# VinAIResearch/COMBAT

Hardware: AMD Instinct MI355X
Metric: images/sec per alternated generator+surrogate step, CIFAR-10 bs=128, 1/2/4/8 GPU (higher is better)
Workload: dtype bf16; 1 GPU; train_generator.py --dataset cifar10 --pc 0.5 --noise_rate 0.08: alternated PreActResNet18 surrogate + UNet generator step (Phase C + Phase G, both Nesterov-SGD updates), bs=128 per GPU, on-device augmentation on; per_gpu_batch=128, global_batch=128, parallelism=dp1 (RCCL all-reduce of netC grads in Phase C, netG grads in Phase G), losses_finite=True, deterministic=True

## Files before the change

combat_amd/_lib.py:

```python
from __future__ import annotations

import ctypes as C
import os

HERE = os.path.dirname(os.path.abspath(__file__))
LIB_PATH = os.environ.get("COMBAT_HIP_LIB") or os.path.join(HERE, "libcombat_hip.so")

c_i32, c_i64, c_f32, c_vp = C.c_int32, C.c_int64, C.c_float, C.c_void_p


class ConvArgs(C.Structure):

    _fields_ = [
        ("N", c_i32), ("H", c_i32), ("W", c_i32), ("C", c_i32),
        ("P", c_i32), ("Q", c_i32), ("K", c_i32),
        ("R", c_i32), ("S", c_i32), ("stride", c_i32), ("pad", c_i32),
        ("mode", c_i32),
        ("src", c_vp), ("wpack", c_vp), ("kpad", c_i32), ("rows_pad", c_i32), ("dst", c_vp),
        ("pro_scale", c_vp), ("pro_shift", c_vp), ("pro_group_stride", c_i32), ("pro_act", c_i32),
        ("pro_slope", c_f32),
        ("bias", c_vp), ("add_pre", c_vp), ("mask_x", c_vp), ("mask_scale", c_vp), ("mask_shift", c_vp),
        ("mask_activated", c_i32), ("mask_group_stride", c_i32), ("mask_slope", c_f32), ("mask_mul_scale", c_i32),
        ("add_post", c_vp), ("tanh_out", c_i32),
        ("stats_kind", c_i32), ("stats", c_vp), ("xh_mean", c_vp), ("xh_rstd", c_vp),
        ("act_dst", c_vp), ("act_scale", c_vp), ("act_shift", c_vp), ("act_slope", c_f32),
        ("workspace", c_vp), ("workspace_bytes", c_i64),
        ("tile", c_i32),
        ("src2", c_vp), ("wpack2", c_vp), ("kpad2", c_i32), ("rows_pad2", c_i32),
        ("pro_act_dst", c_vp),
    ]


class WgradArgs(C.Structure):

    _fields_ = [
        ("N", c_i32), ("H", c_i32), ("W", c_i32), ("C", c_i32),
        ("P", c_i32), ("Q", c_i32), ("K", c_i32),
        ("R", c_i32), ("S", c_i32), ("stride", c_i32), ("pad", c_i32),
        ("src", c_vp), ("dy", c_vp), ("dw", c_vp), ("k_real", c_i32), ("c_real", c_i32),
        ("pro_scale", c_vp), ("pro_shift", c_vp), ("pro_group_stride", c_i32), ("pro_act", c_i32),
        ("pro_slope", c_f32), ("split", c_i32),
        ("workspace", c_vp), ("workspace_bytes", c_i64),
        ("defer_reduce", c_i32), ("reserved", c_i32),
        ("reduce_first", c_vp),
# ... 13 lines not shown
    _fields_ = [("gamma", c_vp), ("beta", c_vp), ("running_mean", c_vp), ("running_var", c_vp),
                ("scale", c_vp), ("shift", c_vp), ("C", c_i32), ("reserved", c_i32)]


SIGNATURES = {
    "combat_version": (C.c_char_p, []),
    "combat_abi_version": (C.c_int, []),
    "combat_set_deterministic": (None, [C.c_int]),
    "combat_get_deterministic": (C.c_int, []),
    "combat_conv_gemm": (C.c_int, [C.POINTER(ConvArgs), c_vp]),
    "combat_conv_gemm_pair": (C.c_int, [C.POINTER(ConvArgs), C.POINTER(ConvArgs), c_vp]),
    "combat_conv_workspace_bytes": (c_i64, [C.POINTER(ConvArgs)]),
    "combat_conv_pick_tile": (C.c_int, [C.POINTER(ConvArgs)]),
    "combat_conv_stats_granule": (C.c_int, [C.c_int]),
    "combat_conv_stats_layout": (C.c_int, [C.POINTER(ConvArgs), C.POINTER(c_i32), C.POINTER(c_i32)]),
    "combat_conv_wgrad": (C.c_int, [C.POINTER(WgradArgs), c_vp]),
    "combat_conv_wgrad_workspace_bytes": (c_i64, [C.POINTER(WgradArgs)]),
    "combat_conv_wgrad_reduce": (C.c_int, [C.POINTER(WgradArgs), c_vp]),
    "combat_pack_weights": (C.c_int, [c_vp, c_i32, c_i32, c_i32, c_i32, c_i32, c_vp, c_i32, c_i32, c_vp, c_i32,
                                      c_i32, c_vp]),
    "combat_norm_finalize": (C.c_int, [c_vp, c_i32, c_i32, c_i32, c_f32, c_f32, c_vp, c_vp, c_vp, c_vp, c_vp, c_vp,
                                       c_vp, c_vp, c_f32, c_vp, c_vp, c_i64, c_vp]),
    "combat_norm_scratch_bytes": (c_i64, [c_i32, c_i32]),
    "combat_bn_eval_fold": (C.c_int, [c_vp, c_vp, c_vp, c_vp, c_f32, c_i32, c_vp, c_vp, c_vp]),
    "combat_pack_weights_batch": (C.c_int, [c_vp, c_i32, c_vp]),
    "combat_bn_eval_fold_batch": (C.c_int, [c_vp, c_i32, c_f32, c_vp]),
    "combat_group_stats": (C.c_int, [c_vp, c_i32, c_i32, c_i32, c_vp, c_vp]),
    "combat_norm_bwd_finalize": (C.c_int, [c_vp, c_i32, c_i32, c_i32, c_f32, c_vp, c_vp, c_vp, c_vp, c_vp, c_vp,
                                           c_vp, c_vp, c_vp, c_i64, c_vp]),
    "combat_norm_bwd_apply": (C.c_int, [c_vp, c_vp, c_vp, c_vp, c_i64, c_i32, c_i32, c_i32, c_vp, c_vp, c_vp, c_vp]),
# ... 101 lines not shown
```

combat_amd/csrc/conv3x3_dma.hip:

```cpp
#include "conv_dma_epilogue.hpp"
#include <stdlib.h>

#ifdef COMBAT_STAMPS
static unsigned long long *g_stamps_dma_host = nullptr;
extern "C" int combat_debug_set_stamps_dma(void *p) { g_stamps_dma_host = (unsigned long long *)p; return 0; }
#define DSTAMP(k)                                                                                        \
    do {                                                                                                 \
        if (threadIdx.x == 0 && p.stamps) p.stamps[blockIdx.x * 16 + (k)] = __builtin_readcyclecounter(); \
        if (threadIdx.x == 0 && p.stamps && ((k) == 0 || (k) == 4)) p.stamps[blockIdx.x * 16 + 8 + (k)] = wall_clock64(); \
    } while (0)
#else
#define DSTAMP(k)
#endif

namespace {

typedef __attribute__((address_space(3))) void lds_void_t;

#if defined(COMBAT_ABL_NODMA)
#define ABL_DMA(x) 0
#else
#define ABL_DMA(x) (x)
#endif

// ... 453 lines not shown
    if constexpr (!WIDE) {
#ifndef COMBAT_ABL_NOTOUCH
        if constexpr (FLX >= 0) epi_touch<TE>(epi);
#endif
        block_barrier();
#ifdef COMBAT_ABL_NOEPI
        {
            float s = 0.f;
#pragma unroll
            for (int i = 0; i < T::FN; ++i)
#pragma unroll
                for (int j = 0; j < T::FM; ++j) s += acc[i][j][0] + acc[i][j][1] + acc[i][j][2] + acc[i][j][3];
            if (s == 12345.678f) reinterpret_cast<float *>(const_cast<void *>(a.dst))[lane] = s;
        }
#else
        if constexpr (FLX >= 0)
            epi_finish_fl<TE, kEpiFlavours[FLX < 0 ? 0 : FLX]>(epi, smem, acc, a, dst_bytes, lane, wid, n0, (long)tile_m * NW + wid, ragged,
                                                                 p.PQ, nullptr, EpiNoHook(), NW);
        else
            epi_finish<TE>(epi, smem, acc, a, dst_bytes, lane, wid, n0, (long)tile_m * NW + wid, ragged, p.PQ, p.flavour, NW);
#endif
    } else {
        epi_init<TE>(epi, lane, wid, n0, [&](int row) -> long { return tile_row_off(wid * 64 + (row - wid * 32)); });
        epi_fetch<TE>(epi, a, dst_bytes, lane, n0);
        block_barrier();
        f32x4_t half[T::FN][2];
#pragma unroll
        for (int i = 0; i < T::FN; ++i) {
            half[i][0] = acc[i][0];
            half[i][1] = acc[i][1];
        }
        epi_finish<TE>(epi, smem, half, a, dst_bytes, lane, wid, n0, ((long)tile_m * NW + wid) * 2, ragged, p.PQ, p.flavour);
// ... 7 lines not shown
        epi_finish<TE>(epi, smem, half, a, dst_bytes, lane, wid, n0, ((long)tile_m * NW + wid) * 2 + 1, ragged, p.PQ, p.flavour);
    }
    DSTAMP(4);
}

template <int BN, int TW, int HB, int NW, int RPW>
__global__ __launch_bounds__(64 * NW, NW == 8 || (RPW == 64 && HB == 2) ? 1 : 2)
void conv3x3_dma_kernel(const DmaParams p) {
    conv3x3_dma_body<BN, TW, HB, NW, RPW>(p);
}

template <int BN, int TW, int HB, int FLX>
__global__ __launch_bounds__(256, 2)
void conv3x3_dma_pro_kernel(const DmaParams p) {
    conv3x3_dma_body<BN, TW, HB, 4, 32, true, FLX>(p);
}

template <int FLI>
__device__ __forceinline__ void conv3x3_ws_body(const DmaParams &p) {
    constexpr int FL = FLI < 0 ? -1 : kEpiFlavours[FLI < 0 ? 0 : FLI];
    constexpr int BN = 64, TW = 16;
    using T = TileCfg<128, BN, 4>;
    using G = DGeo<TW, 4, 32>;
    using EC = EpiCfg<T>;
    constexpr int WBYTES = 9 * BN * 128, HBYTES = G::HBYTES, HPW = G::HPW, EPI_OFF = WBYTES + 2 * HBYTES;
    constexpr int TAB_OFF = EPI_OFF + EC::LDS_BYTES;
    static_assert(G::TI == 1 && G::TH == 8 && G::HWP == 18, "one 16 x 8 patch of one image per tile");
    extern __shared__ __attribute__((aligned(16))) unsigned char smem[];
    const combat_conv_args &a = p.a;
    const int tid = threadIdx.x, lane = tid & 63;
// ... 369 lines not shown
            return COMBAT_ELAUNCH;
        attr_set = true;
    }
    COMBAT_LAUNCH(kern, dim3(p.tiles_m * p.tiles_n), dim3(256), smem, st, p);
    CB_LAUNCH_CHECK();
    return COMBAT_OK;
}

template <int BN, int TW>
int launch_pro(const DmaParams &p, hipStream_t st) {
    if (p.flavour == 0) return p.nchunks == 1 ? launch_pro_fl<BN, TW, 1, 0>(p, st) : launch_pro_fl<BN, TW, 2, 0>(p, st);
    if (p.flavour == 2) return p.nchunks == 1 ? launch_pro_fl<BN, TW, 1, 2>(p, st) : launch_pro_fl<BN, TW, 2, 2>(p, st);
    return COMBAT_EINVAL;
}

template <int BN, int TW, int NW, int RPW = 32>
int launch(const combat_conv_args *a, hipStream_t st) {
    DmaParams p;
    fill<TW, NW, RPW>(a, BN, p);
    if (a->pro_scale) {
        if constexpr (NW == 4 && RPW == 32) return launch_pro<BN, TW>(p, st);
        else return COMBAT_EINVAL;
    }
    return p.nchunks == 1 ? launch_hb<BN, TW, 1, NW, RPW>(p, st) : launch_hb<BN, TW, 2, NW, RPW>(p, st);
}

int tile_bn(int tile) {
    return tile == COMBAT_TILE_D128x64 || tile == COMBAT_TILE_D256x64 || tile == COMBAT_TILE_D256W64 ? 64
                                                                                                 : (tile == COMBAT_TILE_D128x32 ? 32 : 0);
}
int tile_bm(int tile) { return tile == COMBAT_TILE_D256x64 || tile == COMBAT_TILE_D256W64 ? 256 : 128; }

int geo_th(const combat_conv_args *a, int bm) {
    const int tw = geo_tw(a);
// ... 57 lines not shown

int conv3x3d_pick(const combat_conv_args *a) {
    if (a->tile == COMBAT_TILE_S128x64) return ws_applicable(a) ? a->tile : 0;
    if (a->tile) {
        const int bn = tile_bn(a->tile);
        if (a->pro_scale && tile_bm(a->tile) != 128) return 0;
        if (a->tile == COMBAT_TILE_D256W64 && geo_tw(a) != 16) return 0;
        return bn && applicable(a, bn) && geo_th(a, tile_bm(a->tile)) ? a->tile : 0;
    }
    if (!applicable(a, 64)) return applicable(a, 32) ? COMBAT_TILE_D128x32 : 0;
    if (ws_applicable(a) && !getenv("COMBAT_NO_WS")) return COMBAT_TILE_S128x64;
    const long wgs64 = tiles_m_of(a) * (a->K / 64);
    return wgs64 <= 256 ? COMBAT_TILE_D128x32 : COMBAT_TILE_D128x64;
}

int conv3x3d_stats_layout(const combat_conv_args *a, int tile, int *rows, int *rows_per_image) {
    const bool per_wg = a->stats_kind & COMBAT_STATS_PER_WORKGROUP;
    if (tile == COMBAT_TILE_S128x64) {
        if (per_wg) {
            if (!ws_applicable(a)) return COMBAT_EINVAL;
            int per;
            ws_grid(tiles_m_of(a), per, *rows);
            *rows_per_image = 0;
            return COMBAT_OK;
        }
        tile = COMBAT_TILE_D128x64;
    }
    const int bn = tile_bn(tile);
    if (!bn || !applicable(a, bn)) return COMBAT_EINVAL;
    const int tw = geo_tw(a), bm = tile_bm(tile);
// ... 33 lines not shown
```

combat_amd/csrc/conv_common.hpp:

```cpp
#pragma once
#include "common.hpp"
#include <type_traits>

int conv3x3_pick(const combat_conv_args *a);
int conv3x3_stats_layout(const combat_conv_args *a, int tile, int *rows, int *rows_per_image);
int conv3x3_launch(const combat_conv_args *a, int tile, hipStream_t st);
int conv3x3d_pick(const combat_conv_args *a);
int conv3x3d_stats_layout(const combat_conv_args *a, int tile, int *rows, int *rows_per_image);
int conv3x3d_launch(const combat_conv_args *a, int tile, hipStream_t st);
int conv_gather_dma_bn(const combat_conv_args *a);
bool conv_gather_dma_parity_split(const combat_conv_args *a);
bool conv_c8_ok(const combat_conv_args *a);
int conv_c8_launch(const combat_conv_args *a, hipStream_t st);
bool conv_k8_ok(const combat_conv_args *a);
int conv_k8_launch(const combat_conv_args *a, hipStream_t st);
int conv_gather_dma_launch(const combat_conv_args *a, hipStream_t st);
int conv_gather_dma_pair_launch(const combat_conv_args *a, const combat_conv_args *b, hipStream_t st);
long conv_gather_dma_workspace(const combat_conv_args *a);
int conv_wgrad3x3_try(const combat_wgrad_args *a, hipStream_t st);
int conv_wgrad3x3_dma_try(const combat_wgrad_args *a, hipStream_t st);
long conv_wgrad3x3_dma_workspace(const combat_wgrad_args *a);
int conv_wgrad3x3_dma_reduce(const combat_wgrad_args *a, hipStream_t st);

template <int BM, int BN, int WGM_ = 0>
// ... 194 lines not shown
```

combat_amd/csrc/conv_dma_epilogue.hpp:

```cpp
#pragma once
#include "conv_common.hpp"

constexpr unsigned kDmaOob = 0x40000000u;

typedef __attribute__((address_space(3))) float lds_f32_t;
__device__ __forceinline__ void load8f_lds(const lds_f32_t *p, float (&v)[8]) {
    typedef __attribute__((address_space(3))) f32x4_t lds_f32x4_t;
    const f32x4_t a = *reinterpret_cast<const lds_f32x4_t *>(p);
    const f32x4_t b = *reinterpret_cast<const lds_f32x4_t *>(p + 4);
    v[0] = a[0]; v[1] = a[1]; v[2] = a[2]; v[3] = a[3];
    v[4] = b[0]; v[5] = b[1]; v[6] = b[2]; v[7] = b[3];
}

template <typename T>
struct EpiCfg {
    static constexpr int NC = T::NC;
    static constexpr int EQ = 32 * NC / 64;
    static constexpr int NPF = 3 * EQ + 4;
    static constexpr int EPW = 32 * T::EPS > 64 * 20 ? 32 * T::EPS : 64 * 20;
    static constexpr int LDS_BYTES = 4 * 4 * EPW;
};

template <typename T>
struct EpiRegs {
// ... 43 lines not shown
    asm volatile("" : "+v"(r.t_sc[0]), "+v"(r.t_sc[1]), "+v"(r.t_sh[0]), "+v"(r.t_sh[1]));
}

enum : int {
    EF_PRE = 1,
    EF_POST = 2,
    EF_MASK = 4,
    EF_MASK_TAB = 8,
    EF_MUL_SCALE = 16,
    EF_PER_IMAGE = 32,
    EF_ACT = 64,
    EF_STATS1 = 128,
    EF_STATS2 = 256,
    EF_BIAS = 512,
    EF_NODST = 1024,
};

__host__ __device__ inline int epi_flags_of(const combat_conv_args &a) {
    int f = 0;
    if (a.add_pre) f |= EF_PRE;
    if (a.add_post) f |= EF_POST;
    if (a.mask_x) {
        f |= EF_MASK;
        if (a.mask_scale && !a.mask_activated) f |= EF_MASK_TAB;
        if (a.mask_mul_scale && a.mask_scale) f |= EF_MUL_SCALE;
        if (a.mask_group_stride) f |= EF_PER_IMAGE;
    }
    if (a.act_dst) f |= EF_ACT;
    if ((a.stats_kind & 3) == 1) f |= EF_STATS1;
    if ((a.stats_kind & 3) == 2) f |= EF_STATS2;
    if (a.bias) f |= EF_BIAS;
    if (!a.dst) f |= EF_NODST;
    return f;
}

constexpr int kEpiRuntime = EF_PRE | EF_POST | EF_BIAS | EF_NODST;
constexpr int kEpiFlavours[] = {
    0,
    EF_ACT,
    EF_STATS1,
    EF_MASK | EF_MUL_SCALE,
    EF_MASK | EF_MASK_TAB | EF_STATS2,
};
constexpr int kNumEpiFlavours = sizeof(kEpiFlavours) / sizeof(int);

inline int epi_flavour_of(const combat_conv_args &a) {
    const int f = epi_flags_of(a) & ~kEpiRuntime;
    for (int i = 0; i < kNumEpiFlavours; ++i)
        if (kEpiFlavours[i] == f) return i;
    return -1;
}

struct EpiNoHook {
    __device__ __forceinline__ void operator()() const {}
};

template <typename T, int FL, typename PreStore = EpiNoHook, typename StatSink = EpiNoHook>
__device__ __forceinline__ void epi_finish_fl(EpiRegs<T> &er, unsigned char *smem, const f32x4_t (&acc)[T::FN][T::FM],
                                              const combat_conv_args &a, unsigned dst_bytes, int lane, int wid, int n0,
                                              long stats_row, bool ragged, int PQ, const lds_f32_t *lds_tabs = nullptr,
                                              PreStore pre_store = PreStore(), int wg_waves = 0,
                                              StatSink stat_sink = StatSink()) {
    constexpr int NC = EpiCfg<T>::NC, EQ = EpiCfg<T>::EQ, EPW = EpiCfg<T>::EPW;
    constexpr bool RT = FL < 0;
    const int fl = RT ? epi_flags_of(a) : (FL | (epi_flags_of(a) & kEpiRuntime));
    const bool has_pre = fl & EF_PRE, has_post = fl & EF_POST, has_mask = fl & EF_MASK, mask_tab = fl & EF_MASK_TAB;
    const bool mul_scale = fl & EF_MUL_SCALE, per_image = fl & EF_PER_IMAGE, has_act = fl & EF_ACT;
    const bool kind1 = fl & EF_STATS1, kind2 = fl & EF_STATS2, has_bias = fl & EF_BIAS, has_dst = !(fl & EF_NODST);
    const int fr = lane & 15, fq = lane >> 4, ec = lane % NC, K = a.K;
    const __amdgpu_buffer_rsrc_t r_dst = __builtin_amdgcn_make_buffer_rsrc(a.dst, 0, a.dst ? dst_bytes : 0u, 0x00020000);
    const __amdgpu_buffer_rsrc_t r_act = __builtin_amdgcn_make_buffer_rsrc(a.act_dst, 0, a.act_dst ? dst_bytes : 0u, 0x00020000);
    float *ep = reinterpret_cast<float *>(smem) + wid * EPW;
#pragma unroll
    for (int i = 0; i < T::FN; ++i)
#pragma unroll
        for (int j = 0; j < T::FM; ++j)
            *reinterpret_cast<f32x4_t *>(ep + (j * 16 + fr) * T::EPS + i * 16 + fq * 4) = acc[i][j];
    asm volatile("s_waitcnt lgkmcnt(0)" ::: "memory");

// ... 71 lines not shown
        if (has_act || kind1 || kind2) unpack8v(packed[q], vr);
        if (has_act) {
            float y[8];
#pragma unroll
            for (int e = 0; e < 8; ++e) {
                const float qa = fmaf(vr[e], tsc[e], tsh[e]);
                y[e] = qa > 0.f ? qa : qa * aslope;
            }
            packed_act[q] = pack8v(y);
        }
        if (kind1 || kind2) {
            if (ragged && er.evoff[q] == kDmaOob) {
#pragma unroll
                for (int e = 0; e < 8; ++e) vr[e] = 0.f;
            }
            if (kind2) {
#pragma unroll
                for (int e = 0; e < 8; ++e) {
                    s1[e] += vr[e];
                    s2[e] = fmaf(vr[e], (xm[e] - hmn[e]) * hrs[e], s2[e]);
                }
            } else {
#pragma unroll
                for (int e = 0; e < 8; ++e) {
                    s1[e] += vr[e];
                    s2[e] = fmaf(vr[e], vr[e], s2[e]);
                }
            }
        }
    }
    pre_store();
// ... 1 lines not shown
#pragma unroll
        for (int q = 0; q < EQ; ++q) __builtin_amdgcn_raw_buffer_store_b128(packed[q], r_dst, er.evoff[q], 0, 0);
    }
    if (has_act) {
#pragma unroll
        for (int q = 0; q < EQ; ++q) __builtin_amdgcn_raw_buffer_store_b128(packed_act[q], r_act, er.evoff[q], 0, 0);
    }
    if (kind1 || kind2) {
        constexpr bool kSink = !__is_same(StatSink, EpiNoHook);
        const bool per_wg = (kSink || wg_waves > 0) && (a.stats_kind & COMBAT_STATS_PER_WORKGROUP);
        constexpr int VPL = NC * 16 / 64;
        const int vg = (lane / NC) * VPL;
        float tot[VPL];
#pragma unroll
        for (int u = 0; u < VPL; ++u) tot[u] = 0.f;
        if (stats_row >= 0) {
            float *sp = ep + lane * 20;
            *reinterpret_cast<f32x4_t *>(sp) = f32x4_t{s1[0], s1[1], s1[2], s1[3]};
            *reinterpret_cast<f32x4_t *>(sp + 4) = f32x4_t{s1[4], s1[5], s1[6], s1[7]};
            *reinterpret_cast<f32x4_t *>(sp + 8) = f32x4_t{s2[0], s2[1], s2[2], s2[3]};
            *reinterpret_cast<f32x4_t *>(sp + 12) = f32x4_t{s2[4], s2[5], s2[6], s2[7]};
            asm volatile("s_waitcnt lgkmcnt(0)" ::: "memory");
#pragma unroll
            for (int src = 0; src < 64 / NC; ++src) {
                const float *rp = ep + (src * NC + ec) * 20 + vg;
#pragma unroll
                for (int u = 0; u < VPL; ++u) tot[u] += rp[u];
            }
        }
        if (!per_wg) {
            if (stats_row >= 0) {
                float *orow = a.stats + ((size_t)stats_row * 2 + (vg >> 3)) * K + n + (vg & 7);
#pragma unroll
                for (int u = 0; u < VPL; ++u) orow[u] = tot[u];
            }
        } else if constexpr (kSink) {
            stat_sink(tot);
        } else {
            float *slot = ep + lane * VPL;
#pragma unroll
            for (int u = 0; u < VPL; ++u) slot[u] = tot[u];
            __syncthreads();
            if (wid == 0) {
                float sum[VPL];
#pragma unroll
// ... 30 lines not shown
```

combat_amd/csrc/conv_gemm.hip:

```cpp
#include "conv_common.hpp"
#include "plan.hpp"
#include <stdlib.h>

namespace {

struct ConvParams {
    combat_conv_args a;
    int M;
    int PQ;
    int ntaps;
    int c_shift;
    int s_shift;
    int nkt;
    int tiles_m, tiles_n;
    int psplit;
    int mq;
    int cpt;
};

__device__ __forceinline__ int lds_off(int row, int kchunk) { return row * 128 + ((kchunk ^ ((row >> 1) & 7)) << 4); }

template <int BM, int BN>
__global__ __launch_bounds__(256) void conv_gemm_kernel(const ConvParams p) {
    using T = TileCfg<BM, BN>;
// ... 268 lines not shown
        if (bn) return bn == 64 ? COMBAT_TILE_G128x64 : COMBAT_TILE_G128x32;
        if (a->tile) return 0;
    }
    if (a->tile) return a->tile;
    const long M = (long)a->N * a->P * a->Q;
    if (a->K <= 16) return COMBAT_TILE_128x16;
    if (a->K % 128 != 0) return (M / 128) * ((a->K + 63) / 64) >= 256 ? COMBAT_TILE_128x64 : COMBAT_TILE_64x64;
    if ((M / 128) * (a->K / 128) >= 256) return COMBAT_TILE_128x128;
    if ((M / 64) * (a->K / 128) >= 256) return COMBAT_TILE_64x128;
    return COMBAT_TILE_64x64;
}

}

extern "C" int combat_conv_pick_tile(const combat_conv_args *a) { return a ? pick_tile(a) : COMBAT_EINVAL; }

extern "C" int64_t combat_conv_workspace_bytes(const combat_conv_args *a) {
    if (!a || (a->tile && a->tile != COMBAT_TILE_G128x64 && a->tile != COMBAT_TILE_G128x32)) return 0;
    return (int64_t)conv_gather_dma_workspace(a);
}

extern "C" int combat_conv_stats_granule(int tile) {
    switch (tile) {
        case COMBAT_TILE_H256x64: return 64;
        case COMBAT_TILE_128x128:
        case COMBAT_TILE_128x64:
        case COMBAT_TILE_128x16:
        case COMBAT_TILE_H128x128:
        case COMBAT_TILE_H128x64:
        case COMBAT_TILE_D128x64:
// ... 25 lines not shown
        gran = 128;
    const long M = (long)a->N * a->P * a->Q, PQ = (long)a->P * a->Q;
    *rows = (int)((M + gran - 1) / gran);
    *rows_per_image = (PQ % gran == 0) ? (int)(PQ / gran) : 0;
    const int bm = (tile == COMBAT_TILE_64x64 || tile == COMBAT_TILE_64x128) ? 64 : 128;
    if (tile == COMBAT_TILE_C8) {
    } else if (tile == COMBAT_TILE_G128x64 || tile == COMBAT_TILE_G128x32) {
        if (conv_gather_dma_parity_split(a)) *rows_per_image = 0;
    } else if (parity_split(*a) && (M / 4) % bm == 0) {
        *rows_per_image = 0;
    }
    return COMBAT_OK;
}

static int validate_conv_args(const combat_conv_args *a) {
    if (!a || !a->src || !a->wpack || (!a->dst && !a->act_dst)) return COMBAT_EINVAL;
    if (a->act_dst && (!a->act_scale || !a->act_shift)) return COMBAT_EINVAL;
    if (a->N <= 0 || a->H <= 0 || a->W <= 0 || a->P <= 0 || a->Q <= 0) return COMBAT_EINVAL;
    if (a->C < 8 || a->K < 8 || (a->K & 7)) return COMBAT_EINVAL;
    if (a->R != a->S || (a->R != 1 && a->R != 3)) return COMBAT_EINVAL;
    if (a->stride != 1 && a->stride != 2) return COMBAT_EINVAL;
    if (a->mode != 0 && a->mode != 1) return COMBAT_EINVAL;
    if (a->kpad <= 0 || (a->kpad & 63) || a->kpad < a->R * a->S * a->C) return COMBAT_EINVAL;
    if ((a->pro_scale == nullptr) != (a->pro_shift == nullptr)) return COMBAT_EINVAL;
    if (a->mask_scale && !a->mask_shift) return COMBAT_EINVAL;
    if (a->mask_mul_scale && !a->mask_scale) return COMBAT_EINVAL;
    if ((a->src2 == nullptr) != (a->wpack2 == nullptr)) return COMBAT_EINVAL;
    const int skind = a->stats_kind & 3;
    if (a->stats_kind < 0 || (a->stats_kind & ~(3 | COMBAT_STATS_PER_WORKGROUP)) || skind == 3 || (!skind && a->stats_kind) ||
        (skind && !a->stats))
        return COMBAT_EINVAL;
    if (skind == 2 && (!a->mask_x || !a->xh_mean || !a->xh_rstd)) return COMBAT_EINVAL;
    if (ilog2_exact(a->C) < 0) return COMBAT_EINVAL;
    if ((long)a->N * a->P * a->Q > 0x7fffffffL / 8) return COMBAT_EINVAL;
    return COMBAT_OK;
}

extern "C" int combat_conv_gemm(const combat_conv_args *a, void *stream);

extern "C" int combat_conv_gemm_pair(const combat_conv_args *a, const combat_conv_args *b, void *stream) {
    COMBAT_PLAN_HOOK(combat_conv_gemm_pair, a, b);
    if (validate_conv_args(a) != COMBAT_OK || validate_conv_args(b) != COMBAT_OK) return COMBAT_EINVAL;
    const int ta = pick_tile(a), tb = pick_tile(b);
    const bool gather = (ta == COMBAT_TILE_G128x64 || ta == COMBAT_TILE_G128x32) && ta == tb && !a->src2 && !b->src2;
    if (gather) {
        const int rc = conv_gather_dma_pair_launch(a, b, as_stream(stream));
        if (rc != 1) return rc;
// ... 37 lines not shown
```

combat_amd/engine.py:

```python
from __future__ import annotations

import ctypes
import os
from typing import Dict, List, Optional, Tuple

import torch

from . import ops
from ._lib import STATS_PER_WORKGROUP, TILE_D128x32, TILE_D128x64, TILE_S128x64, CombatHipError, ConvArgs, lib
from .nets import UNET_LAYERS
from .ops import Affine, PackedConv, bf16

BATCH_STATS_ROWS = 0 if os.environ.get("COMBAT_STATS_PER_WAVE") == "1" else STATS_PER_WORKGROUP

f32 = torch.float32


def _p(t):
    return None if t is None else t.data_ptr()


class Plan:

    serial = False
# ... 599 lines not shown
        plan.hold(a, part)
        plan.add(key + ".conv", lib.combat_conv_gemm, ctypes.byref(a))
        one_launch = act_dst is not None or defer
        if not fused and not (one_launch and pq <= self.FUSED_DIRECT_PX):
            g = _pow2_part(pq)
            parts = m // g
            part = slot.buf(key + ".part", (parts, 2, c), f32)
            plan.add(key + ".stats", lib.combat_group_stats, dst.data_ptr(), parts, g, c, part.data_ptr())
            rpg = pq // g
        rm = rv = nbt = None
        if running is not None:
            rm, rv, nbt = running
        plan.hold(gamma, beta, rm, rv, nbt)
        if one_launch:
            st.pending = dict(x=dst, part=part, rpg=rpg if part is not None else 0, pxg=m // groups, key=key,
                              gamma=gamma, beta=beta, rm=rm, rv=rv, nbt=nbt)
            if act_dst is not None:
                self._norm_act(plan, st, act_dst, slope)
            return st
        plan.add(key + ".finalize", lib.combat_norm_finalize, part.data_ptr(), groups, rpg, c, float(m // groups),
                 1e-5, _p(gamma), _p(beta), st.mean.data_ptr(), st.rstd.data_ptr(), st.scale.data_ptr(),
                 st.shift.data_ptr(), _p(rm), _p(rv), 0.1, _p(nbt), self._scratch.data_ptr(),
                 self._scratch.numel() * 4)
        return st

    def _lds_prologue_ok(self, src, pc: PackedConv) -> bool:
        if not FUSED_PROLOGUE or pc.R != 3 or pc.stride != 1:
            return False
        n, h, w, _ = src.shape
        probe = getattr(self, "_pro_probe", None)
        if probe is None:
# ... 2 lines not shown
        a = ConvArgs()
        a.N, a.H, a.W, a.C = src.shape
        a.P, a.Q, a.K = h, w, pc.Kc
        a.R = a.S = 3
        a.stride, a.pad, a.mode = 1, pc.pad, 0
        a.src, a.dst, a.pro_act_dst = src.data_ptr(), src.data_ptr(), src.data_ptr()
        a.wpack, a.kpad, a.rows_pad = pc.wf.data_ptr(), pc.kpad_f, pc.rows_f
        a.pro_scale, a.pro_shift, a.pro_act = probe.scale.data_ptr(), probe.shift.data_ptr(), 1
        return lib.combat_conv_pick_tile(ctypes.byref(a)) in (TILE_D128x64, TILE_D128x32)

    def _norm_act(self, plan: Plan, st: NormState, act_dst, slope: float):
        q = st.pending
        st.pending = None
        x = q["x"]
        plan.hold(x, act_dst, q["part"])
        plan.add(q["key"] + ".finact", lib.combat_norm_act_fused, x.data_ptr(), _p(q["part"]), st.groups, q["rpg"],
                 q["pxg"], st.C, 1e-5, float(slope), _p(q["gamma"]), _p(q["beta"]), st.mean.data_ptr(),
                 st.rstd.data_ptr(), st.scale.data_ptr(), st.shift.data_ptr(), _p(q["rm"]), _p(q["rv"]), 0.1,
                 _p(q["nbt"]), self._scratch.data_ptr(), self._scratch.numel() * 4, act_dst.data_ptr())

    def _dgrad_norm(self, plan: Plan, slot: Slot, key: str, dy, dz, pc: PackedConv, x_pre, st: NormState, *,
                    group_stride: int, slope: float, gamma=None, dgamma=None, dbeta=None, add_pre=None, shortcut=None):
        n, p, q, c = dz.shape
        pq, m = p * q, n * p * q
        groups = st.groups
        mask = Affine(st.scale, st.shift, group_stride, True, slope)
        a = ops.conv_args(dy, dz, pc, 1, add_pre=add_pre, mask_x=x_pre, mask=mask, workspace=plan.workspace(dy.device),
                          shortcut=shortcut)
        a.stats_kind = 2 | (BATCH_STATS_ROWS if groups == 1 else 0)
        a.xh_mean, a.xh_rstd = st.mean.data_ptr(), st.rstd.data_ptr()
        _tile_preference(a)
        rows, rpi = ops.conv_stats_layout(a)
        fused = (groups == 1) or (rpi > 0)
        part, rpg = None, 0
        if fused:
            part = slot.buf(key + ".bpart", (rows, 2, c), f32)
            a.stats = part.data_ptr()
            rpg = rows if groups == 1 else rpi
        else:
            a.stats_kind, a.xh_mean, a.xh_rstd = 0, None, None
        plan.hold(a, part)
        plan.add(key + ".dgrad", lib.combat_conv_gemm, ctypes.byref(a))
        if not fused and pq > self.FUSED_DIRECT_PX:
            part, rpg = self._stats_bwd(plan, slot, key, dz, x_pre, st)
        st.bpending = dict(part=part, rpg=rpg, gamma=gamma, dgamma=dgamma, dbeta=dbeta)

    def _stats_bwd(self, plan: Plan, slot: Slot, key: str, dz, x_pre, st: NormState):
        n, p, q, c = dz.shape
        pq, m = p * q, n * p * q
        g = _pow2_part(pq if st.groups > 1 else m)
        parts = m // g
        part = slot.buf(key + ".bpart", (parts, 2, c), f32)
        ppi = (pq // g) if st.groups > 1 else 0
        plan.add(key + ".bstats", lib.combat_group_stats_bwd, dz.data_ptr(), x_pre.data_ptr(), parts, g, c, ppi,
                 st.mean.data_ptr(), st.rstd.data_ptr(), part.data_ptr())
        return part, (pq // g if st.groups > 1 else parts)

    def _bwd_apply(self, plan: Plan, slot: Slot, key: str, dz, x_pre, dx, st: NormState, add=None):
        n, p, q, c = dz.shape
        pq, m = p * q, n * p * q
        pend = getattr(st, "bpending", None) or dict(part=None, rpg=0, gamma=None, dgamma=None, dbeta=None)
        st.bpending = None
        part, rpg = pend["part"], pend["rpg"]
        pxg = m // st.groups
        if part is None and (st.groups == 1 or pq > self.FUSED_DIRECT_PX):
            part, rpg = self._stats_bwd(plan, slot, key, dz, x_pre, st)
        plan.hold(dz, x_pre, dx, add, part, pend["gamma"], pend["dgamma"], pend["dbeta"])
        plan.add(key + ".bfused", lib.combat_norm_bwd_fused, dz.data_ptr(), x_pre.data_ptr(), _p(add), _p(part),
                 st.groups, rpg, pxg, c, _p(pend["gamma"]), st.mean.data_ptr(), st.rstd.data_ptr(),
                 _p(pend["dgamma"]), _p(pend["dbeta"]), self._scratch.data_ptr(), self._scratch.numel() * 4,
                 dx.data_ptr())




class _BN:
    def __init__(self, eng: "NetEngine", mod: torch.nn.BatchNorm2d, prefix: str):
        self.prefix, self.C = prefix, mod.num_features
        self.gamma, self.beta = mod.weight.data, mod.bias.data
# ... 958 lines not shown
```

include/combat_hip.h:

```cpp
#ifndef COMBAT_HIP_H
#define COMBAT_HIP_H

#include <stdint.h>

#ifdef __cplusplus
extern "C" {
#endif

#define COMBAT_OK 0
#define COMBAT_EINVAL (-1)
#define COMBAT_ELAUNCH (-2)

const char *combat_version(void);
int combat_abi_version(void);

void combat_set_deterministic(int on);
int combat_get_deterministic(void);

typedef struct combat_conv_args {
    int32_t N, H, W, C;
    int32_t P, Q, K;
    int32_t R, S, stride, pad;
    int32_t mode;
    const void *src;
// ... 15 lines not shown
    int32_t mask_mul_scale;
    const void *add_post;
    int32_t tanh_out;
    int32_t stats_kind;
    float *stats;
    const float *xh_mean, *xh_rstd;
    void *act_dst;
    const float *act_scale, *act_shift;
    float act_slope;
    void *workspace;
    int64_t workspace_bytes;
    int32_t tile;
    const void *src2, *wpack2;
    int32_t kpad2, rows_pad2;
    void *pro_act_dst;
} combat_conv_args;

#define COMBAT_STATS_PER_WORKGROUP 4
#define COMBAT_TILE_128x128 1
#define COMBAT_TILE_128x64 2
#define COMBAT_TILE_64x64 3
#define COMBAT_TILE_128x16 4
#define COMBAT_TILE_64x128 5
#define COMBAT_TILE_H256x64 6
#define COMBAT_TILE_H128x128 7
#define COMBAT_TILE_H128x64 8
#define COMBAT_TILE_H64x64 9
#define COMBAT_TILE_D128x64 10
#define COMBAT_TILE_D128x32 11
#define COMBAT_TILE_G128x64 12
#define COMBAT_TILE_G128x32 13
#define COMBAT_TILE_D256x64 14
#define COMBAT_TILE_C8 15
#define COMBAT_TILE_S128x64 17
#define COMBAT_TILE_K8 18
#define COMBAT_TILE_D256W64 16

int combat_conv_gemm(const combat_conv_args *a, void *stream);
int combat_conv_gemm_pair(const combat_conv_args *a, const combat_conv_args *b, void *stream);
int64_t combat_conv_workspace_bytes(const combat_conv_args *a);
int combat_conv_pick_tile(const combat_conv_args *a);
int combat_conv_stats_granule(int tile);
int combat_conv_stats_layout(const combat_conv_args *a, int32_t *rows, int32_t *rows_per_image);

typedef struct combat_wgrad_args {
    int32_t N, H, W, C;
    int32_t P, Q, K;
    int32_t R, S, stride, pad;
    const void *src;
    const void *dy;
    float *dw;
    int32_t k_real;
    int32_t c_real;
    const float *pro_scale, *pro_shift;
    int32_t pro_group_stride;
    int32_t pro_act;
    float pro_slope;
    int32_t split;
// ... 188 lines not shown
```

Measured before the change: 33340 images/sec.

## Fuse InstanceNorm stats, normalize and activation into whole-image conv epilogue

```diff
diff --git a/combat_amd/_lib.py b/combat_amd/_lib.py
--- a/combat_amd/_lib.py
+++ b/combat_amd/_lib.py
@@ -28,6 +28,8 @@
         ("tile", c_i32),
         ("src2", c_vp), ("wpack2", c_vp), ("kpad2", c_i32), ("rows_pad2", c_i32),
         ("pro_act_dst", c_vp),
+        ("ln_act_dst", c_vp), ("ln_mean", c_vp), ("ln_rstd", c_vp), ("ln_scale", c_vp), ("ln_shift", c_vp),
+        ("ln_dx", c_vp), ("ln_eps", c_f32), ("ln_slope", c_f32),
     ]
 
 
@@ -71,6 +73,7 @@
     "combat_conv_pick_tile": (C.c_int, [C.POINTER(ConvArgs)]),
     "combat_conv_stats_granule": (C.c_int, [C.c_int]),
     "combat_conv_stats_layout": (C.c_int, [C.POINTER(ConvArgs), C.POINTER(c_i32), C.POINTER(c_i32)]),
+    "combat_conv_norm_local": (C.c_int, [C.POINTER(ConvArgs)]),
     "combat_conv_wgrad": (C.c_int, [C.POINTER(WgradArgs), c_vp]),
     "combat_conv_wgrad_workspace_bytes": (c_i64, [C.POINTER(WgradArgs)]),
     "combat_conv_wgrad_reduce": (C.c_int, [C.POINTER(WgradArgs), c_vp]),
diff --git a/combat_amd/csrc/conv3x3_dma.hip b/combat_amd/csrc/conv3x3_dma.hip
--- a/combat_amd/csrc/conv3x3_dma.hip
+++ b/combat_amd/csrc/conv3x3_dma.hip
@@ -491,8 +491,11 @@
             if (s == 12345.678f) reinterpret_cast<float *>(const_cast<void *>(a.dst))[lane] = s;
         }
 #else
-        if constexpr (FLX >= 0)
-            epi_finish_fl<TE, kEpiFlavours[FLX < 0 ? 0 : FLX]>(epi, smem, acc, a, dst_bytes, lane, wid, n0, (long)tile_m * NW + wid, ragged,
+        if constexpr (FLX >= 100)
+            epi_finish_fl<TE, FLX == 100 ? kEpiLocalFwd : kEpiLocalBwd, EpiNoHook, EpiNoHook, TW>(
+                epi, smem, acc, a, dst_bytes, lane, wid, n0, (long)tile_m * NW + wid, ragged, p.PQ, nullptr, EpiNoHook(), NW);
+        else if constexpr (FLX >= 0)
+            epi_finish_fl<TE, kEpiFlavours[FLX < 0 || FLX >= kNumEpiFlavours ? 0 : FLX]>(epi, smem, acc, a, dst_bytes, lane, wid, n0, (long)tile_m * NW + wid, ragged,
                                                                  p.PQ, nullptr, EpiNoHook(), NW);
         else
             epi_finish<TE>(epi, smem, acc, a, dst_bytes, lane, wid, n0, (long)tile_m * NW + wid, ragged, p.PQ, p.flavour, NW);
@@ -530,6 +533,13 @@
 __global__ __launch_bounds__(256, 2)
 void conv3x3_dma_pro_kernel(const DmaParams p) {
     conv3x3_dma_body<BN, TW, HB, 4, 32, true, FLX>(p);
+}
+
+template <int BN, int TW, int HB, int DIR>
+__global__ __launch_bounds__(256, 2)
+void conv3x3_dma_ln_kernel(const DmaParams p) {
+    static_assert(DGeo<TW, 4, 32>::WHOLE, "a workgroup owns whole images");
+    conv3x3_dma_body<BN, TW, HB, 4, 32, false, 100 + DIR>(p);
 }
 
 template <int FLI>
@@ -929,10 +939,39 @@
     return COMBAT_EINVAL;
 }
 
+template <int BN, int TW, int HB, int DIR>
+int launch_ln_hb(const DmaParams &p, hipStream_t st) {
+    using G = DGeo<TW, 4, 32>;
+    constexpr int stage = HB * G::HBYTES + 3 * BN * 128 + 1024;
+    constexpr int ep = EpiCfg<TileCfg<128, BN, 4>>::LDS_BYTES * (TW == 4 && DIR == 1 ? 2 : 1);
+    constexpr int smem = stage > ep ? stage : ep;
+    static_assert(2 * smem <= 160 * 1024, "two workgroups per CU");
+    auto kern = conv3x3_dma_ln_kernel<BN, TW, HB, DIR>;
+    static bool attr_set = false;
+    if (!attr_set) {
+        if (hipFuncSetAttribute(reinterpret_cast<const void *>(kern), hipFuncAttributeMaxDynamicSharedMemorySize, smem) != hipSuccess)
+            return COMBAT_ELAUNCH;
+        attr_set = true;
+    }
+    COMBAT_LAUNCH(kern, dim3(p.tiles_m * p.tiles_n), dim3(256), smem, st, p);
+    CB_LAUNCH_CHECK();
+    return COMBAT_OK;
+}
+
+template <int BN, int TW>
+int launch_ln(const DmaParams &p, hipStream_t st) {
+    if (p.a.mode == 0) return p.nchunks == 1 ? launch_ln_hb<BN, TW, 1, 0>(p, st) : launch_ln_hb<BN, TW, 2, 0>(p, st);
+    return p.nchunks == 1 ? launch_ln_hb<BN, TW, 1, 1>(p, st) : launch_ln_hb<BN, TW, 2, 1>(p, st);
+}
+
 template <int BN, int TW, int NW, int RPW = 32>
 int launch(const combat_conv_args *a, hipStream_t st) {
     DmaParams p;
     fill<TW, NW, RPW>(a, BN, p);
+    if (a->ln_act_dst || a->ln_dx) {
+        if constexpr (NW == 4 && RPW == 32 && (TW == 4 || TW == 8)) return conv3x3d_norm_local(a) ? launch_ln<BN, TW>(p, st) : COMBAT_EINVAL;
+        else return COMBAT_EINVAL;
+    }
     if (a->pro_scale) {
         if constexpr (NW == 4 && RPW == 32) return launch_pro<BN, TW>(p, st);
         else return COMBAT_EINVAL;
@@ -1020,6 +1059,15 @@
     return wgs64 <= 256 ? COMBAT_TILE_D128x32 : COMBAT_TILE_D128x64;
 }
 
+bool conv3x3d_norm_local(const combat_conv_args *a) {
+    const int tw = geo_tw(a);
+    if ((tw != 4 && tw != 8) || a->tile == COMBAT_TILE_D256x64 || !(applicable(a, 64) || applicable(a, 32))) return false;
+    if (a->pro_scale || a->pro_act_dst || a->act_dst || a->src2) return false;
+    if (a->mode == 0) return !a->mask_x && (a->stats_kind & 3) != 2;
+    return a->mask_x && a->mask_scale && a->mask_shift && !a->mask_activated && !a->mask_mul_scale &&
+           a->mask_group_stride == a->K && (a->stats_kind & 3) != 1;
+}
+
 int conv3x3d_stats_layout(const combat_conv_args *a, int tile, int *rows, int *rows_per_image) {
     const bool per_wg = a->stats_kind & COMBAT_STATS_PER_WORKGROUP;
     if (tile == COMBAT_TILE_S128x64) {
diff --git a/combat_amd/csrc/conv_common.hpp b/combat_amd/csrc/conv_common.hpp
--- a/combat_amd/csrc/conv_common.hpp
+++ b/combat_amd/csrc/conv_common.hpp
@@ -6,6 +6,7 @@
 int conv3x3_stats_layout(const combat_conv_args *a, int tile, int *rows, int *rows_per_image);
 int conv3x3_launch(const combat_conv_args *a, int tile, hipStream_t st);
 int conv3x3d_pick(const combat_conv_args *a);
+bool conv3x3d_norm_local(const combat_conv_args *a);
 int conv3x3d_stats_layout(const combat_conv_args *a, int tile, int *rows, int *rows_per_image);
 int conv3x3d_launch(const combat_conv_args *a, int tile, hipStream_t st);
 int conv_gather_dma_bn(const combat_conv_args *a);
diff --git a/combat_amd/csrc/conv_dma_epilogue.hpp b/combat_amd/csrc/conv_dma_epilogue.hpp
--- a/combat_amd/csrc/conv_dma_epilogue.hpp
+++ b/combat_amd/csrc/conv_dma_epilogue.hpp
@@ -81,6 +81,7 @@
     EF_STATS2 = 256,
     EF_BIAS = 512,
     EF_NODST = 1024,
+    EF_LOCAL = 2048,
 };
 
 __host__ __device__ inline int epi_flags_of(const combat_conv_args &a) {
@@ -110,6 +111,8 @@
     EF_MASK | EF_MASK_TAB | EF_STATS2,
 };
 constexpr int kNumEpiFlavours = sizeof(kEpiFlavours) / sizeof(int);
+constexpr int kEpiLocalFwd = EF_STATS1 | EF_LOCAL;
+constexpr int kEpiLocalBwd = EF_MASK | EF_MASK_TAB | EF_PER_IMAGE | EF_STATS2 | EF_LOCAL;
 
 inline int epi_flavour_of(const combat_conv_args &a) {
     const int f = epi_flags_of(a) & ~kEpiRuntime;
@@ -122,7 +125,7 @@
     __device__ __forceinline__ void operator()() const {}
 };
 
-template <typename T, int FL, typename PreStore = EpiNoHook, typename StatSink = EpiNoHook>
+template <typename T, int FL, typename PreStore = EpiNoHook, typename StatSink = EpiNoHook, int LTW = 0>
 __device__ __forceinline__ void epi_finish_fl(EpiRegs<T> &er, unsigned char *smem, const f32x4_t (&acc)[T::FN][T::FM],
                                               const combat_conv_args &a, unsigned dst_bytes, int lane, int wid, int n0,
                                               long stats_row, bool ragged, int PQ, const lds_f32_t *lds_tabs = nullptr,
@@ -130,6 +133,9 @@
                                               StatSink stat_sink = StatSink()) {
     constexpr int NC = EpiCfg<T>::NC, EQ = EpiCfg<T>::EQ, EPW = EpiCfg<T>::EPW;
     constexpr bool RT = FL < 0;
+    constexpr bool kLocal = !RT && (FL & EF_LOCAL) != 0, kLocal4 = kLocal && LTW == 4, kLocalBwd = kLocal && (FL & EF_STATS2) != 0;
+    static_assert(!kLocal || LTW == 4 || LTW == 8, "local InstanceNorm: whole-image tiles");
+    float *const ep2 = reinterpret_cast<float *>(smem) + (4 + wid) * EPW;
     const int fl = RT ? epi_flags_of(a) : (FL | (epi_flags_of(a) & kEpiRuntime));
     const bool has_pre = fl & EF_PRE, has_post = fl & EF_POST, has_mask = fl & EF_MASK, mask_tab = fl & EF_MASK_TAB;
     const bool mul_scale = fl & EF_MUL_SCALE, per_image = fl & EF_PER_IMAGE, has_act = fl & EF_ACT;
@@ -231,7 +237,19 @@
 #pragma unroll
                 for (int e = 0; e < 8; ++e) vr[e] = 0.f;
             }
-            if (kind2) {
+            if constexpr (kLocal4) {
+                float *tp = ep + r * T::EPS + ec * 8;
+                *reinterpret_cast<f32x4_t *>(tp) = f32x4_t{vr[0], vr[1], vr[2], vr[3]};
+                *reinterpret_cast<f32x4_t *>(tp + 4) = f32x4_t{vr[4], vr[5], vr[6], vr[7]};
+                if constexpr (kLocalBwd) {
+                    float pr[8];
+#pragma unroll
+                    for (int e = 0; e < 8; ++e) pr[e] = fmaf(vr[e], (xm[e] - hmn[e]) * hrs[e], 0.f);
+                    float *pp = ep2 + r * T::EPS + ec * 8;
+                    *reinterpret_cast<f32x4_t *>(pp) = f32x4_t{pr[0], pr[1], pr[2], pr[3]};
+                    *reinterpret_cast<f32x4_t *>(pp + 4) = f32x4_t{pr[4], pr[5], pr[6], pr[7]};
+                }
+            } else if (kind2) {
 #pragma unroll
                 for (int e = 0; e < 8; ++e) {
                     s1[e] += vr[e];
@@ -263,7 +281,7 @@
         float tot[VPL];
 #pragma unroll
         for (int u = 0; u < VPL; ++u) tot[u] = 0.f;
-        if (stats_row >= 0) {
+        if (!kLocal4 && stats_row >= 0) {
             float *sp = ep + lane * 20;
             *reinterpret_cast<f32x4_t *>(sp) = f32x4_t{s1[0], s1[1], s1[2], s1[3]};
             *reinterpret_cast<f32x4_t *>(sp + 4) = f32x4_t{s1[4], s1[5], s1[6], s1[7]};
@@ -277,7 +295,101 @@
                 for (int u = 0; u < VPL; ++u) tot[u] += rp[u];
             }
         }
-        if (!per_wg) {
+        if constexpr (kLocal) {
+            constexpr int BN = NC * 8, NK = kLocalBwd ? 3 : 2;
+            constexpr int ITEMS = LTW == 4 ? 2 * BN / 64 : 1;
+            const float countf = (float)PQ;
+            double t1[ITEMS], t2[ITEMS];
+            float *cf = ep + 512;
+            if constexpr (LTW == 4) {
+#pragma unroll
+                for (int k = 0; k < ITEMS; ++k) {
+                    const int id = lane + 64 * k, h = id / BN, ch = id % BN;
+                    t1[k] = t2[k] = 0.0;
+#pragma unroll
+                    for (int i = 0; i < 16; ++i) {
+                        const float v = ep[(h * 16 + i) * T::EPS + ch];
+                        t1[k] += (double)v;
+                        if constexpr (kLocalBwd) t2[k] += (double)ep2[(h * 16 + i) * T::EPS + ch];
+                        else t2[k] += (double)fmaf(v, v, 0.f);
+                    }
+                }
+                cf = ep;
+            } else {
+                float *slot = ep + lane * VPL;
+#pragma unroll
+                for (int u = 0; u < VPL; ++u) slot[u] = tot[u];
+                asm volatile("s_waitcnt lgkmcnt(0)" ::: "memory");
+                __builtin_amdgcn_s_barrier();
+                asm volatile("" ::: "memory");
+                const float *p0 = reinterpret_cast<const float *>(smem) + (wid & ~1) * EPW, *p1 = p0 + EPW;
+                const int c = (lane % BN) >> 3, e = lane & 7;
+                const int i1 = ((e / VPL) * NC + c) * VPL + e % VPL, i2 = (((8 + e) / VPL) * NC + c) * VPL + (8 + e) % VPL;
+                t1[0] = (double)p0[i1] + (double)p1[i1];
+                t2[0] = (double)p0[i2] + (double)p1[i2];
+            }
+#pragma unroll
+            for (int k = 0; k < ITEMS; ++k) {
+                const int id = lane + 64 * k, h = LTW == 4 ? id / BN : 0, ch = id % BN;
+                const long img = (stats_row * 32 + h * 16) / PQ;
+                const bool own = id < (LTW == 4 ? 2 : 1) * BN;
+                const bool pub = own && img < a.N && (LTW == 4 || !(wid & 1));
+                const long o = img * K + n0 + ch;
+                float *cp = cf + h * NK * BN + ch;
+                if constexpr (!kLocalBwd) {
+                    const double mean = t1[k] / countf;
+                    double var = t2[k] / countf - mean * mean;
+                    if (var < 0.0) var = 0.0;
+                    const double rstd = 1.0 / sqrt(var + (double)a.ln_eps);
+                    const float fsc = (float)rstd, fsh = (float)(0.0 - mean * rstd);
+                    if (own) {
+                        cp[0] = fsc;
+                        cp[BN] = fsh;
+                    }
+                    if (pub) {
+                        a.ln_mean[o] = (float)mean;
+                        a.ln_rstd[o] = (float)rstd;
+                        a.ln_scale[o] = fsc;
+                        a.ln_shift[o] = fsh;
+                    }
+                } else {
+                    const bool ok = own && img < a.N;
+                    const double mean = ok ? (double)a.xh_mean[o] : 0.0, rstd = ok ? (double)a.xh_rstd[o] : 1.0;
+                    const double m1 = t1[k] / countf, m2 = t2[k] / countf;
+                    if (own) {
+                        cp[0] = (float)rstd;
+                        cp[BN] = (float)(-rstd * rstd * m2);
+                        cp[2 * BN] = (float)(rstd * (mean * rstd * m2 - m1));
+                    }
+                    (void)pub;
+                }
+            }
+            asm volatile("s_waitcnt lgkmcnt(0)" ::: "memory");
+            const float lslope = a.ln_slope;
+            const __amdgpu_buffer_rsrc_t r_out = __builtin_amdgcn_make_buffer_rsrc(kLocalBwd ? a.ln_dx : a.ln_act_dst, 0, dst_bytes, 0x00020000);
+#pragma unroll
+            for (int q = 0; q < EQ; ++q) {
+                const int h = LTW == 4 ? q * 2 / EQ : 0;
+                float k0[8], k1[8], vr[8], y[8];
+                load8f(cf + (h * NK + 0) * BN + ec * 8, k0);
+                load8f(cf + (h * NK + 1) * BN + ec * 8, k1);
+                unpack8v(packed[q], vr);
+                if constexpr (kLocalBwd) {
+                    float k2[8], xm[8];
+                    load8f(cf + (h * NK + 2) * BN + ec * 8, k2);
+                    unpack8v(er.e_x[q], xm);
+#pragma unroll
+                    for (int e = 0; e < 8; ++e) y[e] = fmaf(k0[e], vr[e], fmaf(k1[e], xm[e], k2[e]));
+                } else {
+#pragma unroll
+                    for (int e = 0; e < 8; ++e) {
+                        const float qa = fmaf(vr[e], k0[e], k1[e]);
+                        y[e] = qa > 0.f ? qa : qa * lslope;
+                    }
+                }
+                __builtin_amdgcn_raw_buffer_store_b128(pack8v(y), r_out, er.evoff[q], 0, 0);
+            }
+        } else if (!per_wg) {
             if (stats_row >= 0) {
                 float *orow = a.stats + ((size_t)stats_row * 2 + (vg >> 3)) * K + n + (vg & 7);
 #pragma unroll
diff --git a/combat_amd/csrc/conv_gemm.hip b/combat_amd/csrc/conv_gemm.hip
--- a/combat_amd/csrc/conv_gemm.hip
+++ b/combat_amd/csrc/conv_gemm.hip
@@ -306,6 +306,12 @@
 }
 
 extern "C" int combat_conv_pick_tile(const combat_conv_args *a) { return a ? pick_tile(a) : COMBAT_EINVAL; }
+
+static bool conv_norm_local(const combat_conv_args *a) {
+    const int tile = pick_tile(a);
+    return (tile == COMBAT_TILE_D128x64 || tile == COMBAT_TILE_D128x32) && conv3x3d_norm_local(a);
+}
+extern "C" int combat_conv_norm_local(const combat_conv_args *a) { return a && conv_norm_local(a) ? 1 : 0; }
 
 extern "C" int64_t combat_conv_workspace_bytes(const combat_conv_args *a) {
     if (!a || (a->tile && a->tile != COMBAT_TILE_G128x64 && a->tile != COMBAT_TILE_G128x32)) return 0;
@@ -361,7 +367,7 @@
 }
 
 static int validate_conv_args(const combat_conv_args *a) {
-    if (!a || !a->src || !a->wpack || (!a->dst && !a->act_dst)) return COMBAT_EINVAL;
+    if (!a || !a->src || !a->wpack || (!a->dst && !a->act_dst && !a->ln_dx)) return COMBAT_EINVAL;
     if (a->act_dst && (!a->act_scale || !a->act_shift)) return COMBAT_EINVAL;
     if (a->N <= 0 || a->H <= 0 || a->W <= 0 || a->P <= 0 || a->Q <= 0) return COMBAT_EINVAL;
     if (a->C < 8 || a->K < 8 || (a->K & 7)) return COMBAT_EINVAL;
@@ -378,6 +384,12 @@
         (skind && !a->stats))
         return COMBAT_EINVAL;
     if (skind == 2 && (!a->mask_x || !a->xh_mean || !a->xh_rstd)) return COMBAT_EINVAL;
+    if (a->ln_act_dst || a->ln_dx) {
+        if (skind || !conv_norm_local(a)) return COMBAT_EINVAL;
+        if (a->mode == 0 ? (a->ln_dx || !a->dst || !a->ln_mean || !a->ln_rstd || !a->ln_scale || !a->ln_shift)
+                         : (a->ln_act_dst || !a->xh_mean || !a->xh_rstd))
+            return COMBAT_EINVAL;
+    }
     if (ilog2_exact(a->C) < 0) return COMBAT_EINVAL;
     if ((long)a->N * a->P * a->Q > 0x7fffffffL / 8) return COMBAT_EINVAL;
     return COMBAT_OK;
diff --git a/combat_amd/engine.py b/combat_amd/engine.py
--- a/combat_amd/engine.py
+++ b/combat_amd/engine.py
@@ -637,7 +637,7 @@
         plan.hold(gamma, beta, rm, rv, nbt)
         if one_launch:
             st.pending = dict(x=dst, part=part, rpg=rpg if part is not None else 0, pxg=m // groups, key=key,
-                              gamma=gamma, beta=beta, rm=rm, rv=rv, nbt=nbt)
+                              gamma=gamma, beta=beta, rm=rm, rv=rv, nbt=nbt, conv=a)
             if act_dst is not None:
                 self._norm_act(plan, st, act_dst, slope)
             return st
@@ -670,6 +670,14 @@
         st.pending = None
         x = q["x"]
         plan.hold(x, act_dst, q["part"])
+        a = q.get("conv")
+        if (a is not None and st.groups > 1 and all(q[k] is None for k in ("gamma", "beta", "rm", "rv", "nbt"))
+                and lib.combat_conv_norm_local(ctypes.byref(a))):
+            a.stats_kind, a.stats = 0, None
+            a.ln_act_dst, a.ln_eps, a.ln_slope = act_dst.data_ptr(), 1e-5, float(slope)
+            a.ln_mean, a.ln_rstd = st.mean.data_ptr(), st.rstd.data_ptr()
+            a.ln_scale, a.ln_shift = st.scale.data_ptr(), st.shift.data_ptr()
+            return
         plan.add(q["key"] + ".finact", lib.combat_norm_act_fused, x.data_ptr(), _p(q["part"]), st.groups, q["rpg"],
                  q["pxg"], st.C, 1e-5, float(slope), _p(q["gamma"]), _p(q["beta"]), st.mean.data_ptr(),
                  st.rstd.data_ptr(), st.scale.data_ptr(), st.shift.data_ptr(), _p(q["rm"]), _p(q["rv"]), 0.1,
@@ -699,7 +707,7 @@
         plan.add(key + ".dgrad", lib.combat_conv_gemm, ctypes.byref(a))
         if not fused and pq > self.FUSED_DIRECT_PX:
             part, rpg = self._stats_bwd(plan, slot, key, dz, x_pre, st)
-        st.bpending = dict(part=part, rpg=rpg, gamma=gamma, dgamma=dgamma, dbeta=dbeta)
+        st.bpending = dict(part=part, rpg=rpg, gamma=gamma, dgamma=dgamma, dbeta=dbeta, conv=a, dz=dz)
 
     def _stats_bwd(self, plan: Plan, slot: Slot, key: str, dz, x_pre, st: NormState):
         n, p, q, c = dz.shape
@@ -719,6 +727,15 @@
         st.bpending = None
         part, rpg = pend["part"], pend["rpg"]
         pxg = m // st.groups
+        a = pend.get("conv")
+        if (a is not None and pend["dz"] is dz and add is None and st.groups > 1
+                and all(pend[k] is None for k in ("gamma", "dgamma", "dbeta"))
+                and lib.combat_conv_norm_local(ctypes.byref(a))):
+            a.stats_kind, a.stats = 0, None
+            a.xh_mean, a.xh_rstd = st.mean.data_ptr(), st.rstd.data_ptr()
+            a.dst, a.ln_dx = None, dx.data_ptr()
+            plan.hold(x_pre, dx)
+            return
         if part is None and (st.groups == 1 or pq > self.FUSED_DIRECT_PX):
             part, rpg = self._stats_bwd(plan, slot, key, dz, x_pre, st)
         plan.hold(dz, x_pre, dx, add, part, pend["gamma"], pend["dgamma"], pend["dbeta"])
diff --git a/include/combat_hip.h b/include/combat_hip.h
--- a/include/combat_hip.h
+++ b/include/combat_hip.h
@@ -53,6 +53,10 @@
     const void *src2, *wpack2;
     int32_t kpad2, rows_pad2;
     void *pro_act_dst;
+    void *ln_act_dst;
+    float *ln_mean, *ln_rstd, *ln_scale, *ln_shift;
+    void *ln_dx;
+    float ln_eps, ln_slope;
 } combat_conv_args;
 
 #define COMBAT_STATS_PER_WORKGROUP 4
@@ -81,6 +85,7 @@
 int combat_conv_pick_tile(const combat_conv_args *a);
 int combat_conv_stats_granule(int tile);
 int combat_conv_stats_layout(const combat_conv_args *a, int32_t *rows, int32_t *rows_per_image);
+int combat_conv_norm_local(const combat_conv_args *a);
 
 typedef struct combat_wgrad_args {
     int32_t N, H, W, C;
```

Measured after the change: 33570 images/sec (median of 6 runs). No clear change (+0.7%).
